# topling/toplingdb

Hardware: NVIDIA H100
Metric: compaction_input_kv_MB_per_s (higher is better)
Workload: dtype u8

## Files before the change

toplingdb_b200/csrc/api.cu:

```cuda
#include <cuda_runtime.h>
#include <stdio.h>
#include <stdlib.h>
#include <string.h>

#include <algorithm>
#include <map>
#include <memory>
#include <mutex>
#include <unordered_map>
#include <string>
#include <thread>
#include <vector>

#include "../../include/b200c.h"
#include "inflate_rules.h"
#include "kernels.h"
#include "range_plan.h"
#include "scan.cuh"
#include "sst_host.h"

using namespace b200c;

namespace {

// ... 543 lines not shown
#endif
    if (nfiles == 0 || nfiles > kMaxOutFiles) return fail(B200C_ERR_CUDA, "internal: bad output file count");
    CU(j->blocks.reserve(sizeof(BlockRec) * (nblocks + 1)));
    CU(j->idx_esz.reserve(4 * (nblocks + 1)));
    CU(j->idx_eoff.reserve(8 * (nblocks + 1)));
    CU(j->idx_sep.reserve(sizeof(KeyRec) * (nblocks + 1)));
    W.blocks = j->blocks.as<BlockRec>();
    W.idx_esz = j->idx_esz.as<uint32_t>();
    W.idx_eoff = j->idx_eoff.as<uint64_t>();
    W.idx_sep = j->idx_sep.as<KeyRec>();
    base_off.resize(nfiles + 1);
    uint64_t off = 0;
    for (uint32_t f = 0; f < nfiles; f++) {
      base_off[f] = off;
      uint64_t cap = frs[f].data_size + frs[f].filter_bytes + frs[f].n_blocks * 48 + 64 + 4096;
      off += (cap + 255) & ~255ull;
    }
    base_off[nfiles] = off;
    if (getenv("B200C_DEBUG_LAYOUT") || off > (1ull << 44)) {
      fprintf(stderr, "[b200c] layout: n_out=%llu nblocks=%llu nfiles=%u off=%llu hc=%u etiles=%llu\n", (unsigned long long)n_out,
              (unsigned long long)nblocks, nfiles, (unsigned long long)off, hc, (unsigned long long)etiles);
      for (uint32_t f = 0; f < nfiles && f < 4; f++)
        fprintf(stderr, "[b200c]  file %u: first_entry=%llu n_entries=%llu first_block=%llu n_blocks=%llu data_size=%llu filter_bytes=%llu\n", f,
                (unsigned long long)frs[f].first_entry, (unsigned long long)frs[f].n_entries, (unsigned long long)frs[f].first_block,
                (unsigned long long)frs[f].n_blocks, (unsigned long long)frs[f].data_size, (unsigned long long)frs[f].filter_bytes);
    }
    CU(j->out_buf.reserve(off + 256));
    {
      std::vector<uint64_t> coff(nfiles + 1, 0);
      for (uint32_t f = 0; f < nfiles; f++) coff[f + 1] = coff[f] + (frs[f].n_blocks * 48 + 64) / 1024 + 1;
      CU(j->idx_contrib.reserve(64 * (coff[nfiles] + 1)));
      CU(j->idx_contrib_off.reserve(8 * (nfiles + 1)));
      if (int rc = upload_small(j, j->idx_contrib_off.p, coff.data(), 8 * (nfiles + 1))) return rc;
      W.idx_contrib = j->idx_contrib.as<uint64_t>();
      W.idx_contrib_off = j->idx_contrib_off.as<uint64_t>();
    }
    std::vector<uint8_t*> bases(nfiles);
    for (uint32_t f = 0; f < nfiles; f++) bases[f] = j->out_buf.as<uint8_t>() + base_off[f];
    CU(j->out_base_d.reserve(8 * nfiles));
    if (int rc = upload_small(j, j->out_base_d.p, bases.data(), 8 * nfiles)) return rc;
    uint8_t* const* out_base_d = j->out_base_d.as<uint8_t*>();
    j->kt_begin("encode.blocklist");
    launch_encode_blocklist(mcols, ep, W, etiles, nblocks, err, st);
    j->kt_end();
    CU(cudaEventRecord(j->evx[2], st));
    CU(cudaStreamWaitEvent(j->st2, j->evx[2], 0));
    {
      const size_t slot = j->kt_begin("~encode.filestats+index", j->st2);
      launch_encode_filestats(mcols, W, nfiles, j->sms, j->st2);
      launch_encode_index(mcols, ep, W, nblocks, nfiles, out_base_d, err, j->sms, j->st2, &launches);
      j->kt_end(slot, j->st2);
    }
    CU(cudaEventRecord(j->evx[3], j->st2));
    j->kt_begin("encode.emit");
    launch_encode_emit(mcols, ep, W, nblocks, out_base_d, err, j->sms, st);
    j->kt_end();
    launches += 3;
    if (P.bloom_millibits_per_key) {
      j->kt_begin("encode.bloom_build");
      std::vector<uint64_t> boff(nfiles + 1, 0);
      uint64_t max_fb = 0;
      for (uint32_t f = 0; f < nfiles; f++) {
        boff[f + 1] = boff[f] + frs[f].filter_bytes / 1024 + 1;
        max_fb = std::max<uint64_t>(max_fb, frs[f].filter_bytes);
      }
      CU(j->bloom_contrib.reserve(64 * (boff[nfiles] + 1)));
      CU(j->bloom_contrib_off.reserve(8 * (nfiles + 1)));
      if (int rc = upload_small(j, j->bloom_contrib_off.p, boff.data(), 8 * (nfiles + 1))) return rc;
      launch_bloom_build(j->bloom_hashes.as<uint64_t>(), n_out, W.files, nfiles, (uint32_t)std::min<uint64_t>(max_fb, 0xffffffffull), P.bloom_millibits_per_key, P.checksum,
                         out_base_d, j->bloom_contrib.as<uint64_t>(), j->bloom_contrib_off.as<uint64_t>(), st);
      j->kt_end();
      launches += 3;
    }
    CU(cudaStreamWaitEvent(st, j->evx[3], 0));
    {
      int rc = read_small(j, small, h, W.files, &frs);
      if (rc) return rc;
      if (frs.size() != nfiles) return fail(B200C_ERR_CUDA, "internal: output file count changed");
      rc = map_dev_err((uint32_t)h[kSlotErr]);
      if (rc) return rc;
    }
    j->outputs.resize(nfiles);
    CU(j->pin_tails.reserve((size_t)nfiles * 4096 + 64));
    std::vector<TailCopy> tcs(nfiles);
    for (uint32_t f = 0; f < nfiles; f++) {
      const FileRec& fr = frs[f];
      OutputTailInput ti;
      ti.checksum_type = P.checksum;
      ti.format_version = P.format_version;
      ti.data_size = fr.data_size;
      ti.index_size = fr.index_size;
      ti.filter_size = fr.filter_bytes ? fr.filter_bytes - 5 : 0;
      ti.filter_entries = fr.filter_entries;
      ti.num_entries = fr.n_entries;
      ti.num_deletions = fr.num_deletions;
      ti.raw_key_size = fr.raw_key_size;
      ti.raw_value_size = fr.raw_value_size;
      ti.num_data_blocks = fr.n_blocks;
      ti.index_key_is_user_key = !fr.index_has_seq && P.format_version > 2;
      ti.column_family_id = P.column_family_id;
      ti.column_family_name = j->cf_name;
      ti.db_id = j->db_id;
      ti.db_session_id = j->db_session_id;
      ti.db_host_id = j->db_host_id;
      ti.creation_time = P.creation_time;
      ti.oldest_key_time = P.oldest_key_time;
      ti.file_creation_time = j->fct.empty() ? 0 : j->fct[std::min<size_t>(f, j->fct.size() - 1)];
      ti.orig_file_number = P.first_file_number + f;
// ... 1101 lines not shown
```

toplingdb_b200/csrc/encode.cu:

```cuda
#include <cstdlib>

#include "bloom_rules.h"
#include "common.cuh"
#include "gp_rules.h"
#include "kernels.h"
#include "scan.cuh"

namespace b200c {

constexpr int kTT = kEncTile;
constexpr int kW = kEncTile + kEncHalo;
constexpr int kEncThreads = 256;

__global__ void __launch_bounds__(256)
encode_sizes_kernel(KeyCols m, const unsigned long long* __restrict__ n_dev, uint32_t* __restrict__ esz, uint8_t* __restrict__ eshared,
                    TileStat* __restrict__ tstat, unsigned long long* __restrict__ tprefix, uint32_t* __restrict__ min_s1) {
  const uint64_t n = *n_dev;
  const uint64_t ntiles = (n + kEncTile - 1) / kEncTile;
  uint32_t mn = 0xffffffffu, mxs = 0;
  __shared__ unsigned long long red[5];
  __shared__ uint32_t s_mn, s_mx;
  if (threadIdx.x == 0) {
    s_mn = 0xffffffffu;
    s_mx = 0;
// ... 1068 lines not shown
        const uint64_t sq = tr >> 8;
        smin = sq < smin ? sq : smin;
        smax = sq > smax ? sq : smax;
      }
    };
    if (tA >= tB) {
      scan_entries(f0, f1);
    } else {
      scan_entries(f0, tile_start(tA));
      scan_entries(wk.tprefix[tB - 1] & kVal, f1);
      for (uint64_t t = tA + threadIdx.x; t < tB; t += blockDim.x) {
        const TileStat ts = wk.tstat[t];
        kb += ts.raw_key;
        vb += ts.raw_value;
        nd += ts.deletions;
        smin = ts.smallest_seq < smin ? ts.smallest_seq : smin;
        smax = ts.largest_seq > smax ? ts.largest_seq : smax;
      }
    }
    if (threadIdx.x < 2) {
      const uint64_t i = threadIdx.x == 0 ? f0 : f1 - 1;
      const ulonglong2 p = m.pfx[i];
      const KeyRec kr{p.x, p.y, m.tr[i], meta_ulen(m.meta[i]), 0};
      if (threadIdx.x == 0) wk.files[f].smallest = kr;
      else wk.files[f].largest = kr;
    }
  }
#pragma unroll
  for (int d = 16; d; d >>= 1) {
    kb += __shfl_xor_sync(0xffffffffu, kb, d);
    vb += __shfl_xor_sync(0xffffffffu, vb, d);
    nd += __shfl_xor_sync(0xffffffffu, nd, d);
    const unsigned long long a = __shfl_xor_sync(0xffffffffu, smin, d), b = __shfl_xor_sync(0xffffffffu, smax, d);
    smin = a < smin ? a : smin;
    smax = b > smax ? b : smax;
  }
  if ((threadIdx.x & 31) == 0) {
    atomicAdd(&red[0], kb);
    atomicAdd(&red[1], vb);
    atomicAdd(&red[2], nd);
    atomicMin(&red[3], smin);
    atomicMax(&red[4], smax);
  }
  __syncthreads();
  if (threadIdx.x == 0) {
    wk.files[f].raw_key_size = red[0];
    wk.files[f].raw_value_size = red[1];
    wk.files[f].num_deletions = red[2];
    wk.files[f].smallest_seq = red[3];
    wk.files[f].largest_seq = red[4];
  }
}

constexpr int kEmitWarps = 8;
__device__ __forceinline__ void lane_copy(uint8_t* dst, const uint8_t* src, uint32_t n) {
  for (uint32_t i = 0; i < n; i++) dst[i] = src[i];
}
__device__ __forceinline__ void lane_copy_small(uint8_t* dst, const uint8_t* src, uint32_t n) {
  const uint32_t a = (uint32_t)((uintptr_t)src & 3);
  const uint32_t* ws = reinterpret_cast<const uint32_t*>((uintptr_t)src - a);
  const uint32_t nw = (a + n + 3) >> 2;
  uint32_t w[17];
#pragma unroll
  for (int i = 0; i < 17; i++) w[i] = (uint32_t)i < nw ? __ldg(ws + i) : 0u;
  const uint32_t bs = a * 8;
#pragma unroll
  for (int i = 0; i < 16; i++) {
    if ((uint32_t)(4 * i) < n) {
      const uint32_t v = __funnelshift_r(w[i], w[i + 1], bs);
      dst[4 * i] = (uint8_t)v;
      if ((uint32_t)(4 * i + 1) < n) dst[4 * i + 1] = (uint8_t)(v >> 8);
      if ((uint32_t)(4 * i + 2) < n) dst[4 * i + 2] = (uint8_t)(v >> 16);
      if ((uint32_t)(4 * i + 3) < n) dst[4 * i + 3] = (uint8_t)(v >> 24);
    }
  }
}
__device__ void emit_block_warp(const KeyCols& m, const EncodeParams& ep, const EncodeWork& wk, uint64_t b, uint8_t* const* out_base,
                                uint8_t* slice, uint32_t slice_bytes) {
  const unsigned lane = threadIdx.x & 31;
  const uint32_t R = ep.restart_interval;
  {
    const BlockRec br = wk.blocks[b];
    uint8_t* gdst = out_base[br.file_idx] + br.file_off;
    const uint32_t ne = br.n_entries, nrest = (ne + R - 1) / R;
    uint64_t body = 0;
    for (uint32_t j = lane; j < ne; j += 32) {
      uint64_t e = br.first_entry + j;
      uint32_t s1 = wk.esz[e];
      if (j % R == 0) {
        uint32_t mt = m.meta[e], ks = meta_ulen(mt) + 8;
        s1 = entry_size(0, ks, meta_vlen(mt));
      }
      body += s1;
    }
#pragma unroll
    for (int d = 16; d; d >>= 1) body += __shfl_xor_sync(0xffffffffu, body, d);
    const uint64_t payload = body + 4ull * nrest + 4;
    const bool staged = payload + 5 + 16 <= slice_bytes;
    const uint32_t shift = (uint32_t)((uintptr_t)gdst & 15);
    uint8_t* img = staged ? slice : gdst;
    __syncwarp();
    uint64_t off_base = 0;
    for (uint32_t j0 = 0; j0 < ne; j0 += 32) {
      const uint32_t j = j0 + lane;
      uint32_t sz = 0, sh = 0, ks = 0, vs = 0, ulen = 0;
      uint64_t e = br.first_entry + j, hi = 0, lo = 0, tr = 0, vref = 0;
      if (j < ne) {
// ... 171 lines not shown
    for (int mI = 0; mI < 16; mI++)
      if ((uint32_t)mI < nwords) d32[mI] = __funnelshift_r(w[mI + 1], w[mI + 2], bs);
    last = 1;
  }
  const uint32_t done = head + 4 * nwords, rem = n - done;
  if (rem) {
    const uint32_t k = last + nwords;
    const uint32_t lo = __ldg(ws + k), hi = (k + 1 < nw) ? __ldg(ws + k + 1) : 0u;
    const uint32_t v = __funnelshift_r(lo, hi, bs);
    dst[done] = (uint8_t)v;
    if (rem > 1) dst[done + 1] = (uint8_t)(v >> 8);
    if (rem > 2) dst[done + 2] = (uint8_t)(v >> 16);
  }
}
template <int NW>
__device__ __forceinline__ void store_value_words(uint8_t* dst, const uint32_t* w, uint32_t a, uint32_t n) {
  if (n == 0) return;
  uint32_t head = (4 - (uint32_t)((uintptr_t)dst & 3)) & 3;
  if (head > n) head = n;
  {
    const uint32_t v = __funnelshift_r(w[0], w[1], a * 8);
    if (head > 0) dst[0] = (uint8_t)v;
    if (head > 1) dst[1] = (uint8_t)(v >> 8);
    if (head > 2) dst[2] = (uint8_t)(v >> 16);
  }
  const uint32_t t0 = a + head, bs = (t0 & 3) * 8;
  const uint32_t nwords = (n - head) >> 2;
  uint32_t* d32 = reinterpret_cast<uint32_t*>(dst + head);
  const uint32_t done = head + 4 * nwords, rem = n - done;
  uint32_t tailv = 0;
  if ((t0 >> 2) == 0) {
#pragma unroll
    for (int mI = 0; mI < NW - 1; mI++) {
      const uint32_t v = __funnelshift_r(w[mI], w[mI + 1], bs);
      if ((uint32_t)mI < nwords) d32[mI] = v;
      if ((uint32_t)mI == nwords) tailv = v;
    }
  } else {
#pragma unroll
    for (int mI = 0; mI < NW - 1; mI++) {
      const uint32_t v = __funnelshift_r(w[mI + 1], mI + 2 <= NW ? w[mI + 2] : 0u, bs);
      if ((uint32_t)mI < nwords) d32[mI] = v;
      if ((uint32_t)mI == nwords) tailv = v;
    }
  }
  if (rem) {
    dst[done] = (uint8_t)tailv;
    if (rem > 1) dst[done + 1] = (uint8_t)(tailv >> 8);
    if (rem > 2) dst[done + 2] = (uint8_t)(tailv >> 16);
  }
}
constexpr int kEmitPerLane = 3;
constexpr int kEmitMaxEntries = 32 * kEmitPerLane;
template <int kMinCtas>
__global__ void __launch_bounds__(kEmitWarps * 32, kMinCtas)
encode_emit_kernel(KeyCols m, EncodeParams ep, EncodeWork wk, uint64_t nblocks, uint8_t* const* __restrict__ out_base,
                   uint32_t slot_bytes, uint32_t* __restrict__ err) {
  extern __shared__ __align__(128) uint8_t smem[];
  __shared__ XxhLaneTab s_xtab;
  const unsigned lane = threadIdx.x & 31, w = threadIdx.x >> 5;
  uint8_t* const slot = smem + (size_t)w * slot_bytes;
  fill_xxh_lane_tab(&s_xtab);
  __syncthreads();
  const uint32_t xtab = (uint32_t)__cvta_generic_to_shared(&s_xtab);
  const uint32_t R = ep.restart_interval;
  const uint32_t rmask = (R & (R - 1)) == 0 ? R - 1 : 0xffffffffu;
  const uint64_t stride = (uint64_t)gridDim.x * kEmitWarps;
  for (uint64_t b = (uint64_t)blockIdx.x * kEmitWarps + w; b < nblocks; b += stride) {
    const BlockRec br = wk.blocks[b];
    const uint32_t E = br.n_entries;
    const uint64_t e0 = br.first_entry;
    uint8_t* const gdst = out_base[br.file_idx] + br.file_off;
    const uint32_t shift = (uint32_t)((uintptr_t)gdst & 15);
    uint8_t* const img = slot + shift;
    if (E > (uint32_t)kEmitMaxEntries) {
      if (lane == 0) bulk_wait_read0();
      __syncwarp();
      emit_block_warp(m, ep, wk, b, out_base, slot, slot_bytes);
      continue;
    }
    uint32_t sz[kEmitPerLane], pk[kEmitPerLane], vs[kEmitPerLane];
    uint64_t vrf[kEmitPerLane];
    uint32_t tsum = 0;
    {
      uint32_t mtv[kEmitPerLane], shv[kEmitPerLane];
#pragma unroll
      for (int i = 0; i < kEmitPerLane; i++) {
        const uint32_t x = lane * kEmitPerLane + i;
        mtv[i] = 0;
        shv[i] = 0;
        vrf[i] = 0;
        if (x < E) {
          mtv[i] = m.meta[e0 + x];
          shv[i] = wk.eshared[e0 + x];
          vrf[i] = m.vref[e0 + x];
        }
      }
#pragma unroll
      for (int i = 0; i < kEmitPerLane; i++) {
        const uint32_t x = lane * kEmitPerLane + i;
        sz[i] = pk[i] = vs[i] = 0;
        if (x < E) {
          const bool restart = (rmask != 0xffffffffu ? (x & rmask) : (x % R)) == 0;
          const uint32_t ul = meta_ulen(mtv[i]);
          vs[i] = meta_vlen(mtv[i]);
          const uint32_t sh = restart ? 0 : shv[i];
          pk[i] = sh | (ul << 8) | (restart ? 1u << 16 : 0);
          sz[i] = entry_size(sh, ul + 8, vs[i]);
          tsum += sz[i];
        }
      }
    }
    const uint64_t inc = warp_incl_scan64(tsum);
    const uint64_t body64 = __shfl_sync(0xffffffffu, inc, 31);
    const uint32_t nrest = (E + R - 1) / R;
    if (body64 + 4ull * nrest + 4 + 5 + 32 + 16 > slot_bytes) {
      if (lane == 0) bulk_wait_read0();
      __syncwarp();
      emit_block_warp(m, ep, wk, b, out_base, slot, slot_bytes);
      continue;
    }
    if (lane == 0) bulk_wait_read0();
    __syncwarp();
    const uint32_t body = (uint32_t)body64;
    uint32_t off[kEmitPerLane];
    {
      uint32_t run = (uint32_t)(inc - tsum);
#pragma unroll
      for (int i = 0; i < kEmitPerLane; i++) {
        off[i] = run;
        run += sz[i];
      }
    }
    uint32_t voff[kEmitPerLane];
    {
      ulonglong2 ppv[kEmitPerLane];
      uint64_t trv[kEmitPerLane];
#pragma unroll
      for (int i = 0; i < kEmitPerLane; i++) {
        const uint32_t x = lane * kEmitPerLane + i;
        ppv[i] = make_ulonglong2(0, 0);
        trv[i] = 0;
        if (x < E) {
          ppv[i] = m.pfx[e0 + x];
          trv[i] = m.tr[e0 + x];
        }
      }
#pragma unroll
      for (int i = 0; i < kEmitPerLane; i++) {
        const uint32_t x = lane * kEmitPerLane + i;
        voff[i] = 0;
        if (x < E) {
          const uint32_t sh = pk[i] & 0xff, ul = (pk[i] >> 8) & 0xff;
          uint8_t* p = img + off[i];
          const uint32_t ks = ul + 8;
          uint64_t S0, S1, S2;
          key_suffix_words(ppv[i].x, ppv[i].y, ul, trv[i], sh, &S0, &S1, &S2);
          if ((sh | (ks - sh) | vs[i]) < 128) {
            const uint64_t hdr = (uint64_t)sh | ((uint64_t)(ks - sh) << 8) | ((uint64_t)vs[i] << 16);
            const uint64_t W0 = hdr | (S0 << 24), W1 = (S0 >> 40) | (S1 << 24), W2 = (S1 >> 40) | (S2 << 24), W3 = S2 >> 40;
            const uint32_t wv[8] = {(uint32_t)W0, (uint32_t)(W0 >> 32), (uint32_t)W1, (uint32_t)(W1 >> 32),
                                    (uint32_t)W2, (uint32_t)(W2 >> 32), (uint32_t)W3, 0u};
            store_stream28(p, wv, 3 + ks - sh);
            p += 3 + ks - sh;
          } else {
            p += put_varint(p, sh);
            p += put_varint(p, ks - sh);
            p += put_varint(p, vs[i]);
            store_bytes24(p, S0, S1, S2, ks - sh);
            p += ks - sh;
          }
          voff[i] = (uint32_t)(p - img);
          if (pk[i] >> 16) {
            uint8_t* rp = img + body + 4u * (rmask != 0xffffffffu ? x >> __popc(rmask) : x / R);
            rp[0] = (uint8_t)off[i];
            rp[1] = (uint8_t)(off[i] >> 8);
            rp[2] = (uint8_t)(off[i] >> 16);
            rp[3] = (uint8_t)(off[i] >> 24);
          }
        }
      }
    }
    {
      constexpr int kNW = 9;
      bool all_short = true;
#pragma unroll
      for (int i = 0; i < kEmitPerLane; i++) all_short = all_short && vs[i] <= 32;
      if (all_short) {
        uint32_t vw[kEmitPerLane][kNW + 1];
#pragma unroll
        for (int i = 0; i < kEmitPerLane; i++) {
          const uint32_t a = (uint32_t)(vrf[i] & 3);
          const uint32_t* wsrc = reinterpret_cast<const uint32_t*>((uintptr_t)vrf[i] - a);
          const uint32_t nw = vs[i] ? (a + vs[i] + 3) >> 2 : 0;
#pragma unroll
          for (int k = 0; k < kNW; k++) vw[i][k] = (uint32_t)k < nw ? __ldg(wsrc + k) : 0u;
          vw[i][kNW] = 0;
        }
#pragma unroll
        for (int i = 0; i < kEmitPerLane; i++) store_value_words<kNW>(img + voff[i], vw[i], (uint32_t)(vrf[i] & 3), vs[i]);
      } else {
#pragma unroll
        for (int i = 0; i < kEmitPerLane; i++)
          if (vs[i] && vs[i] <= 64) copy_value_small(img + voff[i], (const uint8_t*)(uintptr_t)vrf[i], vs[i]);
      }
    }
#pragma unroll
    for (int i = 0; i < kEmitPerLane; i++) {
      unsigned big = __ballot_sync(0xffffffffu, vs[i] > 64);
      while (big) {
        const int sl = __ffs(big) - 1;
        big &= big - 1;
        const uint32_t vl = __shfl_sync(0xffffffffu, vs[i], sl);
        const uint32_t vo = __shfl_sync(0xffffffffu, voff[i], sl);
        const uint64_t vrr = __shfl_sync(0xffffffffu, vrf[i], sl);
        const uint8_t* sp = (const uint8_t*)(uintptr_t)vrr;
        uint8_t* dp = img + vo;
        const uint32_t a = (uint32_t)((uintptr_t)sp & 3);
        const uint32_t* wsrc = reinterpret_cast<const uint32_t*>((uintptr_t)sp - a);
        const uint32_t nwords = (vl + 3) >> 2;
        for (uint32_t k = lane; k < nwords; k += 32) {
          const uint32_t v = __funnelshift_r(__ldg(wsrc + k), __ldg(wsrc + k + 1), a * 8);
          const uint32_t o = 4 * k;
          dp[o] = (uint8_t)v;
          if (o + 1 < vl) dp[o + 1] = (uint8_t)(v >> 8);
          if (o + 2 < vl) dp[o + 2] = (uint8_t)(v >> 16);
          if (o + 3 < vl) dp[o + 3] = (uint8_t)(v >> 24);
        }
      }
    }
    const uint32_t payload = body + 4 * nrest + 4;
    if (lane == 0) {
      uint8_t* fp = img + body + 4u * nrest;
      fp[0] = (uint8_t)nrest;
      fp[1] = (uint8_t)(nrest >> 8);
      fp[2] = (uint8_t)(nrest >> 16);
      fp[3] = (uint8_t)(nrest >> 24);
    }
    __syncwarp();
    const uint32_t ck = staged_block_checksum(ep.checksum, (uint32_t)__cvta_generic_to_shared(img), img, payload, 0, xtab, lane);
    __syncwarp();
    if (lane == 0) {
      uint8_t* tp = img + payload;
      tp[0] = 0;
      tp[1] = (uint8_t)ck;
      tp[2] = (uint8_t)(ck >> 8);
      tp[3] = (uint8_t)(ck >> 16);
      tp[4] = (uint8_t)(ck >> 24);
    }
    fence_async_smem();
    __syncwarp();
    const uint32_t total = payload + 5;
    uint32_t head = shift ? 16 - shift : 0;
    if (head > total) head = total;
    const uint32_t mid = (total - head) & ~15u;
    if (lane == 0 && mid) bulk_s2g(gdst + head, (uint32_t)__cvta_generic_to_shared(img + head), mid);
    if (lane < head) gdst[lane] = img[lane];
    const uint32_t done = head + mid;
    if (done + lane < total) gdst[done + lane] = img[done + lane];
  }
  if (lane == 0) asm volatile("cp.async.bulk.wait_group 0;" ::: "memory");
  (void)err;
}

__global__ void encode_index_sep_kernel(KeyCols m, EncodeWork wk, uint64_t nblocks) {
  for (uint64_t b = blockIdx.x * (uint64_t)blockDim.x + threadIdx.x; b < nblocks; b += (uint64_t)gridDim.x * blockDim.x) {
    const BlockRec br = wk.blocks[b];
    const uint64_t le = br.first_entry + br.n_entries - 1;
    ulonglong2 lp = m.pfx[le];
    uint32_t lul = meta_ulen(m.meta[le]);
    KeyRec sep{lp.x, lp.y, m.tr[le], lul, 0};
    const bool has_next = b + 1 < nblocks && wk.blocks[b + 1].file_idx == br.file_idx;
    if (has_next) {
      const uint64_t ne = le + 1;
      ulonglong2 np = m.pfx[ne];
      uint32_t nul = meta_ulen(m.meta[ne]);
      if (np.x == lp.x && np.y == lp.y && nul == lul) {
        atomicOr(&wk.files[br.file_idx].index_has_seq, 1u);
      } else {
        uint8_t s[kMaxUserKey], l[kMaxUserKey];
        for (uint32_t t = 0; t < lul; t++) s[t] = (uint8_t)ikey_byte(lp.x, lp.y, lul, 0, t);
        for (uint32_t t = 0; t < nul; t++) l[t] = (uint8_t)ikey_byte(np.x, np.y, nul, 0, t);
        uint32_t minl = lul < nul ? lul : nul, d = 0, tn = lul;
        while (d < minl && s[d] == l[d]) d++;
        bool changed = false;
        if (d < minl && s[d] < l[d]) {
          if (d < nul - 1 || (uint32_t)s[d] + 1 < (uint32_t)l[d]) {
            s[d]++;
            tn = d + 1;
            changed = true;
          } else {
            d++;
            while (d < tn) {
              if (s[d] < 0xff) {
                s[d]++;
                tn = d + 1;
                changed = true;
                break;
              }
              d++;
            }
          }
        }
        if (changed) {
          uint64_t hi = 0, lo = 0;
          for (uint32_t t = 0; t < 8; t++) hi = (hi << 8) | (t < tn ? s[t] : 0);
          for (uint32_t t = 8; t < 16; t++) lo = (lo << 8) | (t < tn ? s[t] : 0);
          sep = KeyRec{hi, lo, (kMaxSeq << 8) | 0x16, tn, 1};
        }
      }
    }
    wk.idx_sep[b] = sep;
// ... 396 lines not shown
  if (ntiles == 0) return;
  static PerDeviceFlag attr;
  const uint64_t dev_bit = attr.bit_of_current_device();
  if (!attr.is_set(dev_bit)) {
    cudaFuncSetAttribute(encode_tables_kernel<uint32_t>, cudaFuncAttributeMaxDynamicSharedMemorySize, (int)sizeof(TablesSmem<uint32_t>));
    cudaFuncSetAttribute(encode_tables_kernel<uint64_t>, cudaFuncAttributeMaxDynamicSharedMemorySize, (int)sizeof(TablesSmem<uint64_t>));
    attr.set(dev_bit);
  }
  if (((uint64_t)max_s1 + 64) * (uint64_t)(kW + 1) < (1ull << 32))
    encode_tables_kernel<uint32_t><<<(unsigned)ntiles, kEncThreads, sizeof(TablesSmem<uint32_t>), st>>>(m, ep, w, m.n, hc, w.nxt, w.disk, err);
  else
    encode_tables_kernel<uint64_t><<<(unsigned)ntiles, kEncThreads, sizeof(TablesSmem<uint64_t>), st>>>(m, ep, w, m.n, hc, w.nxt, w.disk, err);
}
void launch_encode_stitch(KeyCols m, EncodeParams ep, EncodeWork w, uint64_t ntiles, uint32_t hc, uint32_t* err, uint32_t attempt,
                          uint32_t* sflag, cudaStream_t st, uint64_t* launches) {
  if (ntiles == 0) return;
  static const bool solo = !(getenv("B200C_STITCH_SOLO") && atoi(getenv("B200C_STITCH_SOLO")) == 0);
  if (attempt == 1 && !solo) return;
  static PerDeviceFlag attr;
  const uint64_t dev_bit = attr.bit_of_current_device();
  constexpr size_t kSolo = 200 * 1024;
  if (!attr.is_set(dev_bit)) {
    cudaFuncSetAttribute(encode_stitch_kernel, cudaFuncAttributeMaxDynamicSharedMemorySize, (int)kSolo);
    attr.set(dev_bit);
  }
  const size_t fixed = (sizeof(StitchSmem) + 15) & ~(size_t)15;
  uint32_t cache_bytes = 16 * 1024;
  while (cache_bytes < hc * (uint32_t)sizeof(TileRow)) cache_bytes *= 2;
  size_t smem = fixed + 2 * (size_t)cache_bytes;
  if (attempt == 1) {
    const uint32_t big = (uint32_t)(((kSolo - fixed) / 2) & ~(size_t)15);
    if (big > cache_bytes) cache_bytes = big;
    smem = kSolo;
  }
  encode_stitch_kernel<<<1, kEncThreads, smem, st>>>(m, ep, w, m.n, ntiles, hc, cache_bytes, err, attempt, sflag, 300000u);
  if (launches) *launches += 1;
}
void launch_encode_tilestate(KeyCols m, EncodeWork w, uint64_t ntiles, uint32_t hc, uint32_t* err, cudaStream_t st, uint64_t* launches) {
  if (ntiles == 0) return;
  const uint64_t ngroups = (ntiles + kEncGroup - 1) / kEncGroup;
  encode_tilestate_kernel<<<(unsigned)((ngroups + 63) / 64), 64, 0, st>>>(w, m.n, ntiles, hc, err);
  if (launches) *launches += 1;
}
void launch_encode_blocklist(KeyCols m, EncodeParams ep, EncodeWork w, uint64_t ntiles, uint64_t nblk_cap, uint32_t* err,
                             cudaStream_t st) {
  if (ntiles == 0) return;
  encode_blocklist_kernel<<<(unsigned)ntiles, kEncThreads, 0, st>>>(m, ep, w, m.n, nblk_cap, err);
}
void launch_encode_filestats(KeyCols m, EncodeWork w, uint32_t nfiles, int sms, cudaStream_t st) {
  if (m.n == 0 || nfiles == 0) return;
  (void)sms;
  encode_filestats_kernel<<<nfiles, 256, 0, st>>>(m, w, nfiles);
}
uint32_t encode_emit_slice(uint32_t block_size) {
  uint32_t s = block_size + block_size / 4 + 512;
  s = (s + 255) & ~255u;
  if (s < 5632) s = 5632;
  if (s > 24 * 1024) s = 24 * 1024;
  return s;
}
void launch_encode_emit(KeyCols m, EncodeParams ep, EncodeWork w, uint64_t nblocks, uint8_t* const* out_base, uint32_t* err, int sms,
                        cudaStream_t st) {
  if (nblocks == 0) return;
  static int occ = 0;
  if (!occ) {
    const char* e = getenv("B200C_EMIT_CTAS_PER_SM");
    occ = e && atoi(e) >= 3 && atoi(e) <= 5 ? atoi(e) : 4;
  }
  static PerDeviceFlag attr;
  const uint64_t dev_bit = attr.bit_of_current_device();
  if (!attr.is_set(dev_bit)) {
    cudaFuncSetAttribute(encode_emit_kernel<5>, cudaFuncAttributeMaxDynamicSharedMemorySize, 224 * 1024);
    cudaFuncSetAttribute(encode_emit_kernel<3>, cudaFuncAttributeMaxDynamicSharedMemorySize, 224 * 1024);
    cudaFuncSetAttribute(encode_emit_kernel<4>, cudaFuncAttributeMaxDynamicSharedMemorySize, 224 * 1024);
    attr.set(dev_bit);
  }
  const uint32_t slot = encode_emit_slice(ep.block_size);
  const size_t smem = (size_t)slot * kEmitWarps;
  unsigned per_sm = (unsigned)((228 * 1024) / (smem + 1024 + 2048));
  if (per_sm < 1) per_sm = 1;
  if (per_sm > (unsigned)occ) per_sm = (unsigned)occ;
  const uint64_t want = (nblocks + kEmitWarps - 1) / kEmitWarps;
  static const int reserve = getenv("B200C_EMIT_RESERVE") ? atoi(getenv("B200C_EMIT_RESERVE")) : 0;
  uint64_t cap = (uint64_t)sms * per_sm;
  if (reserve > 0 && cap > 4 * (uint64_t)reserve) cap -= (uint64_t)reserve;
  const unsigned grid = (unsigned)(want < cap ? want : cap);
  if (occ == 4) encode_emit_kernel<4><<<grid, kEmitWarps * 32, smem, st>>>(m, ep, w, nblocks, out_base, slot, err);
  else if (occ == 5) encode_emit_kernel<5><<<grid, kEmitWarps * 32, smem, st>>>(m, ep, w, nblocks, out_base, slot, err);
  else encode_emit_kernel<3><<<grid, kEmitWarps * 32, smem, st>>>(m, ep, w, nblocks, out_base, slot, err);
}
void launch_encode_index(KeyCols m, EncodeParams ep, EncodeWork w, uint64_t nblocks, uint32_t nfiles, uint8_t* const* out_base,
                         uint32_t* err, int sms, cudaStream_t st, uint64_t* launches) {
  (void)err;
  if (nblocks == 0) return;
  unsigned g = (unsigned)((nblocks + 255) / 256);
  if (g > (unsigned)sms * 8) g = (unsigned)sms * 8;
  encode_index_sep_kernel<<<g, 256, 0, st>>>(m, w, nblocks);
  encode_index_size_kernel<<<g, 256, 0, st>>>(w, nblocks, ep.format_version);
  exclusive_scan<uint32_t>(w.idx_esz, w.idx_eoff, nblocks, w.scan_tmp, nullptr, st, launches);
  encode_index_write_kernel<<<g, 256, 0, st>>>(w, nblocks, ep.format_version, out_base);
  if (ep.checksum == 4) {
    encode_index_contrib_kernel<<<dim3(64, nfiles), 256, 0, st>>>(w, nfiles, out_base, w.idx_contrib, w.idx_contrib_off);
    if (launches) *launches += 1;
  }
  encode_index_cksum_kernel<<<(nfiles + 3) / 4, 128, 0, st>>>(w, nfiles, ep.checksum, out_base, w.idx_contrib, w.idx_contrib_off);
  if (launches) *launches += 4;
}
void launch_block_checksums(uint32_t type, const uint8_t* data, const uint64_t* offsets, uint32_t n, uint8_t last_byte, uint32_t* out,
                            cudaStream_t st) {
  if (n == 0) return;
  block_checksums_kernel<<<(n + 3) / 4, 128, 0, st>>>(type, data, offsets, n, last_byte, out);
}

}
```

toplingdb_b200/csrc/kernels.h:

```cpp
#pragma once
#include <cuda_runtime.h>
#include <stdint.h>

#include <atomic>

#include "common.cuh"
#include "gp_rules.h"

namespace b200c {

struct PerDeviceFlag {
  std::atomic<uint64_t> mask{0};
  uint64_t bit_of_current_device() const {
    int d = 0;
    cudaGetDevice(&d);
    return 1ull << (d & 63);
  }
  bool is_set(uint64_t bit) const { return (mask.load(std::memory_order_acquire) & bit) != 0; }
  void set(uint64_t bit) { mask.fetch_or(bit, std::memory_order_release); }
};

struct FileDesc {
  const uint8_t* base;
  uint64_t len;
// ... 125 lines not shown
struct TileRow {
  uint32_t exit;
  uint32_t nblk;
  uint64_t bytes;
};
struct TileState {
  uint64_t entry;
  uint64_t blk;
  uint64_t file_off;
  uint32_t file_idx;
  uint32_t pad;
};
constexpr int kEncTile = 4096;
constexpr int kEncHalo = 2048;
constexpr int kEncGroupTiles = 16;
constexpr uint32_t kMaxOutFiles = 4096;

struct EncodeWork {
  uint32_t* esz;
  uint8_t* eshared;
  TileStat* tstat;
  const unsigned long long* tprefix;
  uint64_t nstat;
  uint32_t* min_s1;
  TileRow* rows;
  TileRow* grows;
  TileState* gstate;
  uint32_t* gflag;
  uint32_t* gdone;
  uint32_t* gready;
  TileState* tstate;
  uint64_t* totals;
  BlockRec* blocks;
  FileRec* files;
  uint32_t* idx_esz;
  uint64_t* idx_eoff;
  KeyRec* idx_sep;
  uint64_t* scan_tmp;
  uint64_t* idx_contrib;
  uint64_t* idx_contrib_off;
  uint16_t* nxt;
  uint32_t* disk;
};
void launch_encode_sizes(KeyCols m, const unsigned long long* n_dev, EncodeWork w, unsigned long long* tprefix_out, uint64_t n_cap, int sms, cudaStream_t st);
void launch_encode_tables(KeyCols m, EncodeParams ep, EncodeWork w, uint64_t ntiles, uint32_t hc, uint32_t max_s1, uint32_t* err,
                          cudaStream_t st);
void launch_encode_stitch(KeyCols m, EncodeParams ep, EncodeWork w, uint64_t ntiles, uint32_t hc, uint32_t* err, uint32_t attempt,
                          uint32_t* sflag, cudaStream_t st, uint64_t* launches);
void launch_encode_tilestate(KeyCols m, EncodeWork w, uint64_t ntiles, uint32_t hc, uint32_t* err, cudaStream_t st, uint64_t* launches);
void launch_encode_blocklist(KeyCols m, EncodeParams ep, EncodeWork w, uint64_t ntiles, uint64_t nblk_cap, uint32_t* err,
                             cudaStream_t st);
void launch_encode_filestats(KeyCols m, EncodeWork w, uint32_t nfiles, int sms, cudaStream_t st);
uint32_t encode_emit_slice(uint32_t block_size);
void launch_encode_emit(KeyCols m, EncodeParams ep, EncodeWork w, uint64_t nblocks, uint8_t* const* out_base, uint32_t* err,
                        int sms, cudaStream_t st);
void launch_encode_index(KeyCols m, EncodeParams ep, EncodeWork w, uint64_t nblocks, uint32_t nfiles, uint8_t* const* out_base,
                         uint32_t* err, int sms, cudaStream_t st, uint64_t* launches);
void launch_block_checksums(uint32_t type, const uint8_t* data, const uint64_t* offsets, uint32_t n, uint8_t last_byte,
                            uint32_t* out, cudaStream_t st);

}
```

Baseline: 222,200.

## Double-buffer emit column loads via bulk async copies and split long-entry kernel

```diff
diff --git a/toplingdb_b200/csrc/api.cu b/toplingdb_b200/csrc/api.cu
--- a/toplingdb_b200/csrc/api.cu
+++ b/toplingdb_b200/csrc/api.cu
@@ -619,8 +619,10 @@
       j->kt_end(slot, j->st2);
     }
     CU(cudaEventRecord(j->evx[3], j->st2));
+    uint64_t data_bytes = 0;
+    for (uint32_t f = 0; f < nfiles; f++) data_bytes += frs[f].data_size;
     j->kt_begin("encode.emit");
-    launch_encode_emit(mcols, ep, W, nblocks, out_base_d, err, j->sms, st);
+    launch_encode_emit(mcols, ep, W, nblocks, out_base_d, data_bytes, err, j->sms, st);
     j->kt_end();
     launches += 3;
     if (P.bloom_millibits_per_key) {
diff --git a/toplingdb_b200/csrc/encode.cu b/toplingdb_b200/csrc/encode.cu
--- a/toplingdb_b200/csrc/encode.cu
+++ b/toplingdb_b200/csrc/encode.cu
@@ -1144,7 +1144,7 @@
   }
 }
 
-constexpr int kEmitWarps = 8;
+constexpr int kEmitWarps = 4;
 __device__ __forceinline__ void lane_copy(uint8_t* dst, const uint8_t* src, uint32_t n) {
   for (uint32_t i = 0; i < n; i++) dst[i] = src[i];
 }
@@ -1422,9 +1422,281 @@
 }
 constexpr int kEmitPerLane = 3;
 constexpr int kEmitMaxEntries = 32 * kEmitPerLane;
-template <int kMinCtas>
-__global__ void __launch_bounds__(kEmitWarps * 32, kMinCtas)
+__device__ __forceinline__ uint32_t emit_entry_key(uint8_t* img, uint32_t off, uint32_t pk, uint32_t vs, uint64_t hi, uint64_t lo, uint64_t tr,
+                                                   uint32_t x, uint32_t body, uint32_t R, uint32_t rmask) {
+  const uint32_t sh = pk & 0xff, ul = (pk >> 8) & 0xff;
+  uint8_t* p = img + off;
+  const uint32_t ks = ul + 8;
+  uint64_t S0, S1, S2;
+  key_suffix_words(hi, lo, ul, tr, sh, &S0, &S1, &S2);
+  if ((sh | (ks - sh) | vs) < 128) {
+    const uint64_t hdr = (uint64_t)sh | ((uint64_t)(ks - sh) << 8) | ((uint64_t)vs << 16);
+    const uint64_t W0 = hdr | (S0 << 24), W1 = (S0 >> 40) | (S1 << 24), W2 = (S1 >> 40) | (S2 << 24), W3 = S2 >> 40;
+    const uint32_t wv[8] = {(uint32_t)W0, (uint32_t)(W0 >> 32), (uint32_t)W1, (uint32_t)(W1 >> 32),
+                            (uint32_t)W2, (uint32_t)(W2 >> 32), (uint32_t)W3, 0u};
+    store_stream28(p, wv, 3 + ks - sh);
+    p += 3 + ks - sh;
+  } else {
+    p += put_varint(p, sh);
+    p += put_varint(p, ks - sh);
+    p += put_varint(p, vs);
+    store_bytes24(p, S0, S1, S2, ks - sh);
+    p += ks - sh;
+  }
+  if (pk >> 16) {
+    uint8_t* rp = img + body + 4u * (rmask != 0xffffffffu ? x >> __popc(rmask) : x / R);
+    rp[0] = (uint8_t)off;
+    rp[1] = (uint8_t)(off >> 8);
+    rp[2] = (uint8_t)(off >> 16);
+    rp[3] = (uint8_t)(off >> 24);
+  }
+  return (uint32_t)(p - img);
+}
+__device__ __forceinline__ void emit_copy_long_value(uint8_t* dp, const uint8_t* sp, uint32_t vl, unsigned lane) {
+  const uint32_t a = (uint32_t)((uintptr_t)sp & 3);
+  const uint32_t* wsrc = reinterpret_cast<const uint32_t*>((uintptr_t)sp - a);
+  const uint32_t nwords = (vl + 3) >> 2;
+  for (uint32_t k0 = 0; k0 < nwords; k0 += 128) {
+    uint32_t lo[4], hi[4];
+#pragma unroll
+    for (int t = 0; t < 4; t++) {
+      const uint32_t k = k0 + lane + 32 * t;
+      lo[t] = k < nwords ? __ldg(wsrc + k) : 0u;
+      hi[t] = k < nwords ? __ldg(wsrc + k + 1) : 0u;
+    }
+#pragma unroll
+    for (int t = 0; t < 4; t++) {
+      const uint32_t k = k0 + lane + 32 * t;
+      if (k < nwords) {
+        const uint32_t v = __funnelshift_r(lo[t], hi[t], a * 8);
+        const uint32_t o = 4 * k;
+        dp[o] = (uint8_t)v;
+        if (o + 1 < vl) dp[o + 1] = (uint8_t)(v >> 8);
+        if (o + 2 < vl) dp[o + 2] = (uint8_t)(v >> 16);
+        if (o + 3 < vl) dp[o + 3] = (uint8_t)(v >> 24);
+      }
+    }
+  }
+}
+__device__ __forceinline__ void emit_block_finish(uint8_t* img, uint8_t* gdst, uint32_t shift, uint32_t body, uint32_t nrest, uint32_t cksum,
+                                                  uint32_t xtab, unsigned lane) {
+  const uint32_t payload = body + 4 * nrest + 4;
+  if (lane == 0) {
+    uint8_t* fp = img + body + 4u * nrest;
+    fp[0] = (uint8_t)nrest;
+    fp[1] = (uint8_t)(nrest >> 8);
+    fp[2] = (uint8_t)(nrest >> 16);
+    fp[3] = (uint8_t)(nrest >> 24);
+  }
+  __syncwarp();
+  const uint32_t ck = staged_block_checksum(cksum, (uint32_t)__cvta_generic_to_shared(img), img, payload, 0, xtab, lane);
+  __syncwarp();
+  if (lane == 0) {
+    uint8_t* tp = img + payload;
+    tp[0] = 0;
+    tp[1] = (uint8_t)ck;
+    tp[2] = (uint8_t)(ck >> 8);
+    tp[3] = (uint8_t)(ck >> 16);
+    tp[4] = (uint8_t)(ck >> 24);
+  }
+  fence_async_smem();
+  __syncwarp();
+  const uint32_t total = payload + 5;
+  uint32_t head = shift ? 16 - shift : 0;
+  if (head > total) head = total;
+  const uint32_t mid = (total - head) & ~15u;
+  if (lane == 0 && mid) bulk_s2g(gdst + head, (uint32_t)__cvta_generic_to_shared(img + head), mid);
+  if (lane < head) gdst[lane] = img[lane];
+  const uint32_t done = head + mid;
+  if (done + lane < total) gdst[done + lane] = img[done + lane];
+}
+constexpr int kEmitCtasPerSm = 3;
+constexpr uint32_t kStPfx = 0, kStTr = kStPfx + 16 * kEmitMaxEntries + 16, kStVref = kStTr + 8 * kEmitMaxEntries + 16,
+                   kStMeta = kStVref + 8 * kEmitMaxEntries + 16, kStEsh = kStMeta + 4 * kEmitMaxEntries + 16,
+                   kStageBytes = kStEsh + kEmitMaxEntries + 16;
+static_assert(kStTr % 16 == 0 && kStVref % 16 == 0 && kStMeta % 16 == 0 && kStEsh % 16 == 0 && kStageBytes % 16 == 0,
+              "bulk copies need 16-byte aligned shared-memory destinations");
+__device__ __forceinline__ uint32_t cover16(const void* p, uint32_t bytes, uintptr_t* a0) {
+  *a0 = (uintptr_t)p & ~(uintptr_t)15;
+  return (uint32_t)((((uintptr_t)p + bytes + 15) & ~(uintptr_t)15) - *a0);
+}
+__device__ __forceinline__ void emit_stage_fill(const KeyCols& m, const EncodeWork& wk, uint64_t e0, uint32_t E, uint32_t stage, uint32_t bar) {
+  uintptr_t a[5];
+  const uint32_t n0 = cover16(m.pfx + e0, 16 * E, &a[0]), n1 = cover16(m.tr + e0, 8 * E, &a[1]), n2 = cover16(m.vref + e0, 8 * E, &a[2]),
+                 n3 = cover16(m.meta + e0, 4 * E, &a[3]), n4 = cover16(wk.eshared + e0, E, &a[4]);
+  mbar_expect_tx(bar, n0 + n1 + n2 + n3 + n4);
+  bulk_g2s(stage + kStPfx, reinterpret_cast<const void*>(a[0]), n0, bar);
+  bulk_g2s(stage + kStTr, reinterpret_cast<const void*>(a[1]), n1, bar);
+  bulk_g2s(stage + kStVref, reinterpret_cast<const void*>(a[2]), n2, bar);
+  bulk_g2s(stage + kStMeta, reinterpret_cast<const void*>(a[3]), n3, bar);
+  bulk_g2s(stage + kStEsh, reinterpret_cast<const void*>(a[4]), n4, bar);
+}
+__global__ void __launch_bounds__(kEmitWarps * 32, kEmitCtasPerSm)
 encode_emit_kernel(KeyCols m, EncodeParams ep, EncodeWork wk, uint64_t nblocks, uint8_t* const* __restrict__ out_base,
+                   uint32_t slot_bytes, uint32_t* __restrict__ err) {
+  extern __shared__ __align__(128) uint8_t smem[];
+  __shared__ XxhLaneTab s_xtab;
+  __shared__ __align__(8) uint64_t s_bar[kEmitWarps][2];
+  const unsigned lane = threadIdx.x & 31, w = threadIdx.x >> 5;
+  uint8_t* const slot = smem + (size_t)w * slot_bytes;
+  uint8_t* const stages = smem + (size_t)kEmitWarps * slot_bytes + (size_t)w * 2 * kStageBytes;
+  const uint32_t stages_sa = (uint32_t)__cvta_generic_to_shared(stages), bar0 = (uint32_t)__cvta_generic_to_shared(&s_bar[w][0]);
+  fill_xxh_lane_tab(&s_xtab);
+  if (lane == 0) {
+    mbar_init(bar0, 1);
+    mbar_init(bar0 + 8, 1);
+    asm volatile("fence.mbarrier_init.release.cluster;" ::: "memory");
+  }
+  __syncthreads();
+  const uint32_t xtab = (uint32_t)__cvta_generic_to_shared(&s_xtab);
+  const uint32_t R = ep.restart_interval;
+  const uint32_t rmask = (R & (R - 1)) == 0 ? R - 1 : 0xffffffffu;
+  const uint64_t stride = (uint64_t)gridDim.x * kEmitWarps;
+  uint64_t b = (uint64_t)blockIdx.x * kEmitWarps + w;
+  BlockRec br{}, brn{}, nbr{}, nbrn{};
+  if (b < nblocks) br = wk.blocks[b];
+  if (b + stride < nblocks) brn = wk.blocks[b + stride];
+  if (lane == 0 && b < nblocks && br.n_entries <= (uint32_t)kEmitMaxEntries) emit_stage_fill(m, wk, br.first_entry, br.n_entries, stages_sa, bar0);
+  uint32_t s = 0, parity = 0;
+  for (; b < nblocks; b += stride, s ^= 1, br = nbr, brn = nbrn) {
+    __syncwarp();
+    if (lane == 0 && b + stride < nblocks && brn.n_entries <= (uint32_t)kEmitMaxEntries) {
+      fence_async_smem();
+      emit_stage_fill(m, wk, brn.first_entry, brn.n_entries, stages_sa + (s ^ 1) * kStageBytes, bar0 + 8 * (s ^ 1));
+    }
+    auto load_next = [&]() {
+      if (b + stride < nblocks) nbr = wk.blocks[b + stride];
+      if (b + 2 * stride < nblocks) nbrn = wk.blocks[b + 2 * stride];
+    };
+    const uint32_t E = br.n_entries;
+    const uint64_t e0 = br.first_entry;
+    uint8_t* const gdst = out_base[br.file_idx] + br.file_off;
+    const uint32_t shift = (uint32_t)((uintptr_t)gdst & 15);
+    uint8_t* const img = slot + shift;
+    if (E > (uint32_t)kEmitMaxEntries) {
+      load_next();
+      if (lane == 0) bulk_wait_read0();
+      __syncwarp();
+      emit_block_warp(m, ep, wk, b, out_base, slot, slot_bytes);
+      continue;
+    }
+    const uint8_t* const stg = stages + s * kStageBytes;
+    const ulonglong2* const c_pfx = reinterpret_cast<const ulonglong2*>(stg + kStPfx + ((uintptr_t)(m.pfx + e0) & 15));
+    const uint64_t* const c_tr = reinterpret_cast<const uint64_t*>(stg + kStTr + ((uintptr_t)(m.tr + e0) & 15));
+    const uint64_t* const c_vref = reinterpret_cast<const uint64_t*>(stg + kStVref + ((uintptr_t)(m.vref + e0) & 15));
+    const uint32_t* const c_meta = reinterpret_cast<const uint32_t*>(stg + kStMeta + ((uintptr_t)(m.meta + e0) & 15));
+    const uint8_t* const c_esh = stg + kStEsh + ((uintptr_t)(wk.eshared + e0) & 15);
+    mbar_wait(bar0 + 8 * s, (parity >> s) & 1);
+    parity ^= 1u << s;
+    uint32_t sz[kEmitPerLane], pk[kEmitPerLane], vs[kEmitPerLane];
+    uint32_t tsum = 0;
+#pragma unroll
+    for (int i = 0; i < kEmitPerLane; i++) {
+      const uint32_t x = lane * kEmitPerLane + i;
+      sz[i] = pk[i] = vs[i] = 0;
+      if (x < E) {
+        const uint32_t mt = c_meta[x];
+        const bool restart = (rmask != 0xffffffffu ? (x & rmask) : (x % R)) == 0;
+        const uint32_t ul = meta_ulen(mt);
+        vs[i] = meta_vlen(mt);
+        const uint32_t sh = restart ? 0 : c_esh[x];
+        pk[i] = sh | (ul << 8) | (restart ? 1u << 16 : 0);
+        sz[i] = entry_size(sh, ul + 8, vs[i]);
+        tsum += sz[i];
+      }
+    }
+    const uint64_t inc = warp_incl_scan64(tsum);
+    const uint64_t body64 = __shfl_sync(0xffffffffu, inc, 31);
+    const uint32_t nrest = (E + R - 1) / R;
+    if (body64 + 4ull * nrest + 4 + 5 + 32 + 16 > slot_bytes) {
+      load_next();
+      if (lane == 0) bulk_wait_read0();
+      __syncwarp();
+      emit_block_warp(m, ep, wk, b, out_base, slot, slot_bytes);
+      continue;
+    }
+    const uint32_t body = (uint32_t)body64;
+    uint32_t off[kEmitPerLane];
+    {
+      uint32_t run = (uint32_t)(inc - tsum);
+#pragma unroll
+      for (int i = 0; i < kEmitPerLane; i++) {
+        off[i] = run;
+        run += sz[i];
+      }
+    }
+    constexpr int kNW = 9;
+    bool all_short = true;
+#pragma unroll
+    for (int i = 0; i < kEmitPerLane; i++) all_short = all_short && vs[i] <= 32;
+    uint4 vc[kEmitPerLane][3];
+    if (all_short) {
+#pragma unroll
+      for (int i = 0; i < kEmitPerLane; i++) {
+        const uint64_t vr = vs[i] ? c_vref[lane * kEmitPerLane + i] : 0;
+        const uint32_t a = (uint32_t)(vr & 15);
+        const uint4* csrc = reinterpret_cast<const uint4*>((uintptr_t)vr - a);
+        const uint32_t nc = vs[i] ? (a + vs[i] + 15) >> 4 : 0;
+#pragma unroll
+        for (int k = 0; k < 3; k++) vc[i][k] = (uint32_t)k < nc ? __ldg(csrc + k) : make_uint4(0, 0, 0, 0);
+      }
+    }
+    if (lane == 0) bulk_wait_read0();
+    __syncwarp();
+    uint32_t voff[kEmitPerLane];
+#pragma unroll
+    for (int i = 0; i < kEmitPerLane; i++) {
+      const uint32_t x = lane * kEmitPerLane + i;
+      voff[i] = 0;
+      if (x < E) {
+        const ulonglong2 pp = c_pfx[x];
+        voff[i] = emit_entry_key(img, off[i], pk[i], vs[i], pp.x, pp.y, c_tr[x], x, body, R, rmask);
+      }
+    }
+    if (all_short) {
+#pragma unroll
+      for (int i = 0; i < kEmitPerLane; i++) {
+        if (!vs[i]) continue;
+        const uint32_t a = (uint32_t)(c_vref[lane * kEmitPerLane + i] & 15);
+        uint32_t w[12] = {vc[i][0].x, vc[i][0].y, vc[i][0].z, vc[i][0].w, vc[i][1].x, vc[i][1].y,
+                          vc[i][1].z, vc[i][1].w, vc[i][2].x, vc[i][2].y, vc[i][2].z, vc[i][2].w};
+        if (a & 8) {
+#pragma unroll
+          for (int k = 0; k < 10; k++) w[k] = w[k + 2];
+        }
+        if (a & 4) {
+#pragma unroll
+          for (int k = 0; k < 11; k++) w[k] = w[k + 1];
+        }
+        w[kNW] = 0;
+        store_value_words<kNW>(img + voff[i], w, a & 3, vs[i]);
+      }
+    } else {
+#pragma unroll
+      for (int i = 0; i < kEmitPerLane; i++)
+        if (vs[i] && vs[i] <= 64) copy_value_small(img + voff[i], (const uint8_t*)(uintptr_t)c_vref[lane * kEmitPerLane + i], vs[i]);
+    }
+#pragma unroll
+    for (int i = 0; i < kEmitPerLane; i++) {
+      unsigned big = __ballot_sync(0xffffffffu, vs[i] > 64);
+      while (big) {
+        const int sl = __ffs(big) - 1;
+        big &= big - 1;
+        const uint32_t vl = __shfl_sync(0xffffffffu, vs[i], sl);
+        const uint32_t vo = __shfl_sync(0xffffffffu, voff[i], sl);
+        emit_copy_long_value(img + vo, (const uint8_t*)(uintptr_t)c_vref[sl * kEmitPerLane + i], vl, lane);
+      }
+    }
+    load_next();
+    emit_block_finish(img, gdst, shift, body, nrest, ep.checksum, xtab, lane);
+  }
+  if (lane == 0) asm volatile("cp.async.bulk.wait_group 0;" ::: "memory");
+  (void)err;
+}
+
+constexpr int kEmitLongWarps = 8, kEmitLongCtasPerSm = 4;
+__global__ void __launch_bounds__(kEmitLongWarps * 32, kEmitLongCtasPerSm)
+encode_emit_long_kernel(KeyCols m, EncodeParams ep, EncodeWork wk, uint64_t nblocks, uint8_t* const* __restrict__ out_base,
                    uint32_t slot_bytes, uint32_t* __restrict__ err) {
   extern __shared__ __align__(128) uint8_t smem[];
   __shared__ XxhLaneTab s_xtab;
@@ -1435,8 +1707,8 @@
   const uint32_t xtab = (uint32_t)__cvta_generic_to_shared(&s_xtab);
   const uint32_t R = ep.restart_interval;
   const uint32_t rmask = (R & (R - 1)) == 0 ? R - 1 : 0xffffffffu;
-  const uint64_t stride = (uint64_t)gridDim.x * kEmitWarps;
-  for (uint64_t b = (uint64_t)blockIdx.x * kEmitWarps + w; b < nblocks; b += stride) {
+  const uint64_t stride = (uint64_t)gridDim.x * kEmitLongWarps;
+  for (uint64_t b = (uint64_t)blockIdx.x * kEmitLongWarps + w; b < nblocks; b += stride) {
     const BlockRec br = wk.blocks[b];
     const uint32_t E = br.n_entries;
     const uint64_t e0 = br.first_entry;
@@ -1521,33 +1793,7 @@
         const uint32_t x = lane * kEmitPerLane + i;
         voff[i] = 0;
         if (x < E) {
-          const uint32_t sh = pk[i] & 0xff, ul = (pk[i] >> 8) & 0xff;
-          uint8_t* p = img + off[i];
-          const uint32_t ks = ul + 8;
-          uint64_t S0, S1, S2;
-          key_suffix_words(ppv[i].x, ppv[i].y, ul, trv[i], sh, &S0, &S1, &S2);
-          if ((sh | (ks - sh) | vs[i]) < 128) {
-            const uint64_t hdr = (uint64_t)sh | ((uint64_t)(ks - sh) << 8) | ((uint64_t)vs[i] << 16);
-            const uint64_t W0 = hdr | (S0 << 24), W1 = (S0 >> 40) | (S1 << 24), W2 = (S1 >> 40) | (S2 << 24), W3 = S2 >> 40;
-            const uint32_t wv[8] = {(uint32_t)W0, (uint32_t)(W0 >> 32), (uint32_t)W1, (uint32_t)(W1 >> 32),
-                                    (uint32_t)W2, (uint32_t)(W2 >> 32), (uint32_t)W3, 0u};
-            store_stream28(p, wv, 3 + ks - sh);
-            p += 3 + ks - sh;
-          } else {
-            p += put_varint(p, sh);
-            p += put_varint(p, ks - sh);
-            p += put_varint(p, vs[i]);
-            store_bytes24(p, S0, S1, S2, ks - sh);
-            p += ks - sh;
-          }
-          voff[i] = (uint32_t)(p - img);
-          if (pk[i] >> 16) {
-            uint8_t* rp = img + body + 4u * (rmask != 0xffffffffu ? x >> __popc(rmask) : x / R);
-            rp[0] = (uint8_t)off[i];
-            rp[1] = (uint8_t)(off[i] >> 8);
-            rp[2] = (uint8_t)(off[i] >> 16);
-            rp[3] = (uint8_t)(off[i] >> 24);
-          }
+          voff[i] = emit_entry_key(img, off[i], pk[i], vs[i], ppv[i].x, ppv[i].y, trv[i], x, body, R, rmask);
         }
       }
     }
@@ -1584,50 +1830,10 @@
         const uint32_t vl = __shfl_sync(0xffffffffu, vs[i], sl);
         const uint32_t vo = __shfl_sync(0xffffffffu, voff[i], sl);
         const uint64_t vrr = __shfl_sync(0xffffffffu, vrf[i], sl);
-        const uint8_t* sp = (const uint8_t*)(uintptr_t)vrr;
-        uint8_t* dp = img + vo;
-        const uint32_t a = (uint32_t)((uintptr_t)sp & 3);
-        const uint32_t* wsrc = reinterpret_cast<const uint32_t*>((uintptr_t)sp - a);
-        const uint32_t nwords = (vl + 3) >> 2;
-        for (uint32_t k = lane; k < nwords; k += 32) {
-          const uint32_t v = __funnelshift_r(__ldg(wsrc + k), __ldg(wsrc + k + 1), a * 8);
-          const uint32_t o = 4 * k;
-          dp[o] = (uint8_t)v;
-          if (o + 1 < vl) dp[o + 1] = (uint8_t)(v >> 8);
-          if (o + 2 < vl) dp[o + 2] = (uint8_t)(v >> 16);
-          if (o + 3 < vl) dp[o + 3] = (uint8_t)(v >> 24);
-        }
-      }
-    }
-    const uint32_t payload = body + 4 * nrest + 4;
-    if (lane == 0) {
-      uint8_t* fp = img + body + 4u * nrest;
-      fp[0] = (uint8_t)nrest;
-      fp[1] = (uint8_t)(nrest >> 8);
-      fp[2] = (uint8_t)(nrest >> 16);
-      fp[3] = (uint8_t)(nrest >> 24);
-    }
-    __syncwarp();
-    const uint32_t ck = staged_block_checksum(ep.checksum, (uint32_t)__cvta_generic_to_shared(img), img, payload, 0, xtab, lane);
-    __syncwarp();
-    if (lane == 0) {
-      uint8_t* tp = img + payload;
-      tp[0] = 0;
-      tp[1] = (uint8_t)ck;
-      tp[2] = (uint8_t)(ck >> 8);
-      tp[3] = (uint8_t)(ck >> 16);
-      tp[4] = (uint8_t)(ck >> 24);
-    }
-    fence_async_smem();
-    __syncwarp();
-    const uint32_t total = payload + 5;
-    uint32_t head = shift ? 16 - shift : 0;
-    if (head > total) head = total;
-    const uint32_t mid = (total - head) & ~15u;
-    if (lane == 0 && mid) bulk_s2g(gdst + head, (uint32_t)__cvta_generic_to_shared(img + head), mid);
-    if (lane < head) gdst[lane] = img[lane];
-    const uint32_t done = head + mid;
-    if (done + lane < total) gdst[done + lane] = img[done + lane];
+        emit_copy_long_value(img + vo, (const uint8_t*)(uintptr_t)vrr, vl, lane);
+      }
+    }
+    emit_block_finish(img, gdst, shift, body, nrest, ep.checksum, xtab, lane);
   }
   if (lane == 0) asm volatile("cp.async.bulk.wait_group 0;" ::: "memory");
   (void)err;
@@ -2130,6 +2336,7 @@
   (void)sms;
   encode_filestats_kernel<<<nfiles, 256, 0, st>>>(m, w, nfiles);
 }
+constexpr uint32_t kEmitMaxSmem = 224 * 1024;
 uint32_t encode_emit_slice(uint32_t block_size) {
   uint32_t s = block_size + block_size / 4 + 512;
   s = (s + 255) & ~255u;
@@ -2137,35 +2344,31 @@
   if (s > 24 * 1024) s = 24 * 1024;
   return s;
 }
-void launch_encode_emit(KeyCols m, EncodeParams ep, EncodeWork w, uint64_t nblocks, uint8_t* const* out_base, uint32_t* err, int sms,
-                        cudaStream_t st) {
+static_assert(kEmitWarps * (24 * 1024 + 2 * kStageBytes) <= kEmitMaxSmem, "the largest slots and their column stages fit one CTA");
+void launch_encode_emit(KeyCols m, EncodeParams ep, EncodeWork w, uint64_t nblocks, uint8_t* const* out_base, uint64_t data_bytes,
+                        uint32_t* err, int sms, cudaStream_t st) {
   if (nblocks == 0) return;
-  static int occ = 0;
-  if (!occ) {
-    const char* e = getenv("B200C_EMIT_CTAS_PER_SM");
-    occ = e && atoi(e) >= 3 && atoi(e) <= 5 ? atoi(e) : 4;
-  }
   static PerDeviceFlag attr;
   const uint64_t dev_bit = attr.bit_of_current_device();
   if (!attr.is_set(dev_bit)) {
-    cudaFuncSetAttribute(encode_emit_kernel<5>, cudaFuncAttributeMaxDynamicSharedMemorySize, 224 * 1024);
-    cudaFuncSetAttribute(encode_emit_kernel<3>, cudaFuncAttributeMaxDynamicSharedMemorySize, 224 * 1024);
-    cudaFuncSetAttribute(encode_emit_kernel<4>, cudaFuncAttributeMaxDynamicSharedMemorySize, 224 * 1024);
+    cudaFuncSetAttribute(encode_emit_kernel, cudaFuncAttributeMaxDynamicSharedMemorySize, kEmitMaxSmem);
+    cudaFuncSetAttribute(encode_emit_long_kernel, cudaFuncAttributeMaxDynamicSharedMemorySize, kEmitMaxSmem);
     attr.set(dev_bit);
   }
+  const bool long_entries = data_bytes > 64 * m.n;
+  const int warps = long_entries ? kEmitLongWarps : kEmitWarps, ctas = long_entries ? kEmitLongCtasPerSm : kEmitCtasPerSm;
   const uint32_t slot = encode_emit_slice(ep.block_size);
-  const size_t smem = (size_t)slot * kEmitWarps;
-  unsigned per_sm = (unsigned)((228 * 1024) / (smem + 1024 + 2048));
+  const size_t smem = (size_t)warps * (slot + (long_entries ? 0 : 2 * kStageBytes));
+  int per_sm = 0;
+  cudaOccupancyMaxActiveBlocksPerMultiprocessor(&per_sm, long_entries ? (const void*)encode_emit_long_kernel : (const void*)encode_emit_kernel,
+                                                warps * 32, smem);
   if (per_sm < 1) per_sm = 1;
-  if (per_sm > (unsigned)occ) per_sm = (unsigned)occ;
-  const uint64_t want = (nblocks + kEmitWarps - 1) / kEmitWarps;
-  static const int reserve = getenv("B200C_EMIT_RESERVE") ? atoi(getenv("B200C_EMIT_RESERVE")) : 0;
-  uint64_t cap = (uint64_t)sms * per_sm;
-  if (reserve > 0 && cap > 4 * (uint64_t)reserve) cap -= (uint64_t)reserve;
+  if (per_sm > ctas) per_sm = ctas;
+  const uint64_t want = (nblocks + warps - 1) / warps;
+  const uint64_t cap = (uint64_t)sms * per_sm;
   const unsigned grid = (unsigned)(want < cap ? want : cap);
-  if (occ == 4) encode_emit_kernel<4><<<grid, kEmitWarps * 32, smem, st>>>(m, ep, w, nblocks, out_base, slot, err);
-  else if (occ == 5) encode_emit_kernel<5><<<grid, kEmitWarps * 32, smem, st>>>(m, ep, w, nblocks, out_base, slot, err);
-  else encode_emit_kernel<3><<<grid, kEmitWarps * 32, smem, st>>>(m, ep, w, nblocks, out_base, slot, err);
+  if (long_entries) encode_emit_long_kernel<<<grid, warps * 32, smem, st>>>(m, ep, w, nblocks, out_base, slot, err);
+  else encode_emit_kernel<<<grid, warps * 32, smem, st>>>(m, ep, w, nblocks, out_base, slot, err);
 }
 void launch_encode_index(KeyCols m, EncodeParams ep, EncodeWork w, uint64_t nblocks, uint32_t nfiles, uint8_t* const* out_base,
                          uint32_t* err, int sms, cudaStream_t st, uint64_t* launches) {
diff --git a/toplingdb_b200/csrc/kernels.h b/toplingdb_b200/csrc/kernels.h
--- a/toplingdb_b200/csrc/kernels.h
+++ b/toplingdb_b200/csrc/kernels.h
@@ -201,8 +201,8 @@
                              cudaStream_t st);
 void launch_encode_filestats(KeyCols m, EncodeWork w, uint32_t nfiles, int sms, cudaStream_t st);
 uint32_t encode_emit_slice(uint32_t block_size);
-void launch_encode_emit(KeyCols m, EncodeParams ep, EncodeWork w, uint64_t nblocks, uint8_t* const* out_base, uint32_t* err,
-                        int sms, cudaStream_t st);
+void launch_encode_emit(KeyCols m, EncodeParams ep, EncodeWork w, uint64_t nblocks, uint8_t* const* out_base, uint64_t data_bytes,
+                        uint32_t* err, int sms, cudaStream_t st);
 void launch_encode_index(KeyCols m, EncodeParams ep, EncodeWork w, uint64_t nblocks, uint32_t nfiles, uint8_t* const* out_base,
                          uint32_t* err, int sms, cudaStream_t st, uint64_t* launches);
 void launch_block_checksums(uint32_t type, const uint8_t* data, const uint64_t* offsets, uint32_t n, uint8_t last_byte,
```

New measurement: 240,800, median of 6. 1.08x the previous value.
